# lambdaclass/ethrex

Measured on AMD Instinct MI355X. Metric: bn254_msm_point_adds_per_s, higher is better.
Workload: dtype u64x4_mod_bn254; 1 GPU; bn254_g1_msm_2^24; n_points=16777216, window_c=17, windows=15, signed_digits=True, parallelism=single GPU

## Files before the change

ethrex_amd/csrc/api_msm_bn254.hip:

```cpp
#include "msm_api_impl.h"

extern "C" int ethrex_mi355_msm_plan_create(size_t n, em_msm_plan **plan) {
    return msm_create_t(n, (msm_plan_t<Bn254G1> **)plan);
}
extern "C" int ethrex_mi355_msm_plan_destroy(em_msm_plan *p) {
    return msm_destroy_t((msm_plan_t<Bn254G1> *)p);
}
extern "C" int ethrex_mi355_msm_upload_points(em_msm_plan *p,
                                              const uint8_t *points64) {
    return msm_upload_points_t((msm_plan_t<Bn254G1> *)p, points64);
}
extern "C" int ethrex_mi355_msm_gen_points(em_msm_plan *p, uint64_t start) {
    return msm_gen_points_t((msm_plan_t<Bn254G1> *)p, start);
}
extern "C" int ethrex_mi355_msm_download_points(em_msm_plan *p, uint8_t *out64) {
    return msm_download_points_t((msm_plan_t<Bn254G1> *)p, out64);
}
extern "C" int ethrex_mi355_msm_upload_scalars(em_msm_plan *p,
                                               const uint8_t *scalars32) {
    return msm_upload_scalars_t((msm_plan_t<Bn254G1> *)p, scalars32);
}
extern "C" int ethrex_mi355_msm_run(em_msm_plan *p, uint8_t out[64]) {
    return msm_run_inner_t((msm_plan_t<Bn254G1> *)p, out, 0);
}
// ... 22 lines not shown
extern "C" int ethrex_mi355_msm_fb_info(em_msm_plan *p, int *c,
                                        double *precompute_ms,
                                        uint64_t *table_bytes) {
    if (!p) return EM_ERR_INPUT;
    if (c) *c = p->fb_c;
    if (precompute_ms) *precompute_ms = p->fb_precompute_ms;
    if (table_bytes) *table_bytes = p->fb_table_bytes;
    return EM_OK;
}

extern "C" int ethrex_mi355_msm_download_fb_rows(em_msm_plan *p, int w,
                                                 size_t start, size_t count,
                                                 uint8_t *out64) {
    if (!p || !out64 || !p->fb_c || !p->have_points || w < 0 ||
        w >= (254 + p->fb_c - 1) / p->fb_c || count == 0 || start >= p->n ||
        count > p->n - start)
        return EM_ERR_INPUT;
    int rc0 = msm_sync_t((msm_plan_t<Bn254G1> *)p);
    if (rc0) return rc0;
    hipLaunchKernelGGL(k_points_to_be, dim3(blocks_for(count, 256)), dim3(256),
                       0, 0, p->d_pts_ext + (size_t)w * p->n + start,
                       p->d_inf + start, p->d_scratch, count);
    HIP_TRY(hipMemcpy(out64, p->d_scratch, count * 64, hipMemcpyDeviceToHost));
    return EM_OK;
}

extern "C" int ethrex_mi355_msm_combine(em_msm_plan *p,
                                        const uint8_t *jacobians96,
                                        size_t count, uint8_t out[64]) {
    if (!p || !jacobians96 || !out || count == 0 || count * 96 > p->n * 64)
        return EM_ERR_INPUT;
    HIP_TRY(hipMemcpy(p->d_scratch, jacobians96, 96 * count,
                      hipMemcpyHostToDevice));
    hipLaunchKernelGGL((k_g1_combine<Bn254G1>), dim3(1), dim3(64), 0, 0,
                       p->d_scratch, count, p->sb[0].out);
    HIP_TRY(hipMemcpy(out, p->sb[0].out, 64, hipMemcpyDeviceToHost));
    return EM_OK;
}

extern "C" int ethrex_mi355_bn254_g1_msm(const uint8_t *points64,
                                         const uint8_t *scalars32, size_t n,
                                         uint8_t out[64]) {
    if (!points64 || !scalars32 || !out || n == 0) return EM_ERR_INPUT;
    em_msm_plan *p = nullptr;
    int rc = ethrex_mi355_msm_plan_create(n, &p);
    if (rc) return rc;
// ... 77 lines not shown
```

ethrex_amd/csrc/msm_api_impl.h:

```cpp
#pragma once
#include "em_api_common.h"

#include <rocprim/rocprim.hpp>

#include "../../include/ethrex_mi355.h"
#include "gpu_field.h"
#include "gpu_g1_9.h"
#include "msm_kernels.h"
#include "msm_fbm_partition_kernels.h"

using namespace em;


struct msm_step_bufs {
    uint32_t *keys_out = nullptr;
    uint32_t *vals_out = nullptr;
    uint32_t *offsets = nullptr;
    uint32_t *sched = nullptr;
    uint8_t *out = nullptr;
};

template <typename C>
struct msm_plan_t {
    using F = typename C::F;
    static constexpr int PB = pt_bytes<C>::AFF;
    static constexpr int JB = pt_bytes<C>::JAC;
    static constexpr int AB = PB;
    static constexpr int SB = msm_curve<C>::BN_SCALARS ? 254 : 256;
    size_t n;
    int cbits;
    g1aT<C> *d_pts = nullptr;
    g1aT<C> *d_pts_ext = nullptr;
    bool fixed_base = false;
    int fb_c = 0;
    uint32_t fb_chunk = 0;
    int fb_len_bits = 0;
    double fb_precompute_ms = 0;
    uint64_t fb_table_bytes = 0;
    uint32_t *d_fb_boff = nullptr;
    g1jT<C> *d_fb_slots = nullptr;
    uint32_t fbp_tile = 0;
    uint32_t *d_fbp = nullptr;
    uint8_t *d_inf = nullptr;
    fe4 *d_scalars = nullptr;
    uint8_t *d_scratch = nullptr;
    uint32_t *d_keys = nullptr;
    uint32_t *d_vals = nullptr;
    msm_step_bufs sb[2];
    void *d_sort_tmp = nullptr;
    size_t sort_tmp_bytes = 0;
    uint32_t *d_blen = nullptr;
    uint32_t *d_blen_out = nullptr;
    uint32_t *d_bids = nullptr;
    g1jT<C> *d_buckets = nullptr;
    g1jT<C> *d_seg_sum = nullptr;
    g1jT<C> *d_seg_wsum = nullptr;
    g1jT<C> *d_partials = nullptr;
    g1jT<C> *d_windows = nullptr;
    uint32_t *d_err = nullptr;
    bool use_tree = false;
    int tree_levels = 0;
    g1aT<C> *d_lvl[2] = {nullptr, nullptr};
    feL<F::L> *d_aux = nullptr;
    uint32_t *d_loff[2] = {nullptr, nullptr};
    uint32_t *d_cnt = nullptr;
// ... 21 lines not shown
    int apar = 0;
};

constexpr int NWIN_MAX = 32;

template <typename C>
static int msm_sync_t(msm_plan_t<C> *p);
template <typename C>
static void host_windows_horner(const uint8_t *wire, int nwin, int cbits,
                                uint8_t *out, int out_mode);

template <typename C>
static int msm_destroy_t(msm_plan_t<C> *p) {
    if (!p) return EM_ERR_INPUT;
    if (p->s_comp) {
        (void)hipStreamSynchronize(p->s_sort);
        (void)hipStreamSynchronize(p->s_comp);
    }
    (void)hipFree(p->d_pts);
    (void)hipFree(p->d_pts_ext);
    (void)hipFree(p->d_fb_boff);
    (void)hipFree(p->d_fb_slots);
    (void)hipFree(p->d_fbp);
    (void)hipFree(p->d_inf);
    (void)hipFree(p->d_scalars);
    (void)hipFree(p->d_scratch);
    (void)hipFree(p->d_keys);
    (void)hipFree(p->d_vals);
    (void)hipFree(p->d_sort_tmp);
    (void)hipFree(p->d_blen);
    (void)hipFree(p->d_blen_out);
    (void)hipFree(p->d_bids);
    (void)hipFree(p->d_buckets);
    (void)hipFree(p->d_seg_sum);
    (void)hipFree(p->d_seg_wsum);
    (void)hipFree(p->d_partials);
    (void)hipFree(p->d_windows);
    (void)hipFree(p->d_err);
    (void)hipFree(p->d_lvl[0]);
    (void)hipFree(p->d_lvl[1]);
    (void)hipFree(p->d_aux);
    (void)hipFree(p->d_loff[0]);
    (void)hipFree(p->d_loff[1]);
    (void)hipFree(p->d_cnt);
    (void)hipFree(p->d_scan_tmp);
    for (auto &b : p->sb) {
        (void)hipFree(b.keys_out);
        (void)hipFree(b.vals_out);
        (void)hipFree(b.offsets);
        (void)hipFree(b.sched);
        (void)hipFree(b.out);
    }
    if (p->h_out[0]) (void)hipHostFree(p->h_out[0]);
    if (p->h_out[1]) (void)hipHostFree(p->h_out[1]);
    for (int i = 0; i < 2; i++) {
        if (p->gx_sort[i]) (void)hipGraphExecDestroy(p->gx_sort[i]);
        if (p->gx_comp[i]) (void)hipGraphExecDestroy(p->gx_comp[i]);
    }
    if (p->s_sort) (void)hipStreamDestroy(p->s_sort);
    if (p->s_comp) (void)hipStreamDestroy(p->s_comp);
    delete p;
    return EM_OK;
}

constexpr int FBM_DEFAULT_C = 22;
constexpr size_t FBM_MIN_N = (size_t)1 << 23;

struct fbp_layout {
    size_t cnt_a, cnt_b, off_a, off_b, ucnt, uoff, words;
};
static inline fbp_layout fbp_lay(uint32_t nbuckets) {
    const size_t na = (size_t)(nbuckets >> 16) + 1;
    const size_t nc = (size_t)(nbuckets >> 8) + 1;
    fbp_layout l;
    l.cnt_a = 0;
    l.cnt_b = na;
    l.off_a = na + nc;
    l.off_b = 2 * na + nc;
    l.ucnt = 2 * na + 2 * nc;
    l.uoff = 2 * na + 3 * nc;
    l.words = 2 * na + 4 * nc;
    return l;
}
static inline size_t fbp_words(uint32_t nbuckets) { return fbp_lay(nbuckets).words; }

template <typename FN>
static int fbm_dispatch(int c, FN fn) {
    switch (c) {
    case 20: return fn(CfgFbm20{});
    case 22: return fn(CfgFbm22{});
    case 24: return fn(CfgFbm24{});
    }
    return EM_ERR_INPUT;
}

template <typename C>
static int fbm_select(size_t n) {
    if constexpr (!msm_curve<C>::FB_MERGED) {
        return 0;
    } else {
        int c = 0;
        if (const char *ev = std::getenv("EM_MSM_FB")) {
            c = atoi(ev);
            if (c != 20 && c != 22 && c != 24) return 0;
        } else if (n >= FBM_MIN_N && std::getenv("EM_MSM_TREE") == nullptr) {
            c = FBM_DEFAULT_C;
        } else {
// ... 116 lines not shown
    mal((void **)&p->d_keys, total * kb);
    mal((void **)&p->d_vals, total * 4);
    for (auto &b : p->sb) {
        mal((void **)&b.keys_out, total * kb);
        mal((void **)&b.vals_out, total * 4);
        mal((void **)&b.offsets, (nsched + 1) * 4);
        mal((void **)&b.sched, nsched * 4);
        mal((void **)&b.out, (size_t)NWIN_MAX * msm_plan_t<C>::JB);
    }
    mal((void **)&p->d_blen, nsched * 4);
    mal((void **)&p->d_blen_out, nsched * 4);
    mal((void **)&p->d_bids, nsched * 4);
    mal((void **)&p->d_buckets, (size_t)nbuckets * sizeof(g1jT<C>));
    if constexpr (msm_curve<C>::FB_MERGED) if (p->fb_c) {
        mal((void **)&p->d_fb_boff, ((size_t)nbuckets + 1) * 4);
        mal((void **)&p->d_fb_slots, nsched * sizeof(g1jT<C>));
        mal((void **)&p->d_cnt, ((size_t)nbuckets + 1) * 4);
        mal((void **)&p->d_loff[0], ((size_t)nbuckets + 1) * 4);
        mal((void **)&p->d_loff[1], ((size_t)nbuckets + 1) * 4);
        if (e == hipSuccess)
            e = rocprim::exclusive_scan(nullptr, p->scan_tmp_bytes, p->d_cnt,
                                        p->d_loff[0], 0u,
                                        (size_t)nbuckets + 1);
        if (e == hipSuccess) e = hipMalloc(&p->d_scan_tmp, p->scan_tmp_bytes);
        if (p->fbp_tile) mal((void **)&p->d_fbp, fbp_words(nbuckets) * 4);
    }
    mal((void **)&p->d_seg_sum, (size_t)nseg_tot * sizeof(g1jT<C>));
    mal((void **)&p->d_seg_wsum, (size_t)nseg_tot * sizeof(g1jT<C>));
    mal((void **)&p->d_partials, (size_t)npart * sizeof(g1jT<C>));
    mal((void **)&p->d_windows, (size_t)nwin * sizeof(g1jT<C>));
    mal((void **)&p->d_err, 4);
    if (e == hipSuccess) {
        if (p->keys16)
            e = rocprim::radix_sort_pairs(
                nullptr, p->sort_tmp_bytes, (const uint16_t *)p->d_keys,
                (uint16_t *)p->sb[0].keys_out, p->d_vals, p->sb[0].vals_out,
                n, 0, 16);
        else
            e = rocprim::radix_sort_pairs(
                nullptr, p->sort_tmp_bytes, p->d_keys, p->sb[0].keys_out,
                p->d_vals, p->sb[0].vals_out, total, 0, sort_bits);
        size_t tmp_len = 0;
        if (e == hipSuccess)
            e = rocprim::radix_sort_pairs(nullptr, tmp_len, p->d_blen,
                                          p->d_blen_out, p->d_bids,
                                          p->sb[0].sched, nsched, 0, 32);
        if (tmp_len > p->sort_tmp_bytes) p->sort_tmp_bytes = tmp_len;
        if (e == hipSuccess) e = hipMalloc(&p->d_sort_tmp, p->sort_tmp_bytes);
// ... 290 lines not shown
#define EM_HT(call)                         \
    do {                                    \
        hipError_t _e = (call);             \
        if (_e != hipSuccess) return _e;    \
    } while (0)

template <typename C, typename CFG>
static const g1aT<C> *msm_walk_pts(const msm_plan_t<C> *p) {
    constexpr bool TABLE = std::is_same_v<CFG, CfgFB> || is_fbm<CFG>::value;
    return TABLE ? p->d_pts_ext : p->d_pts;
}

static int msm_split_pct() {
    static int pct = std::getenv("EM_MSM_SPLIT")
                         ? atoi(std::getenv("EM_MSM_SPLIT"))
                         : 0;
    return pct;
}

template <typename C, typename CFG>
static hipError_t fbm_enqueue_partition(msm_plan_t<C> *p, int par,
                                        hipStream_t st) {
    using G = fbp_geom<CFG::IB>;
    const msm_step_bufs &b = p->sb[par];
    const size_t total = p->n * (size_t)CFG::NWIN_REAL;
    const uint32_t T = p->fbp_tile;
    const fbp_layout l = fbp_lay(G::NBUCKETS);
    uint32_t *cnt_a = p->d_fbp + l.cnt_a, *cnt_b = p->d_fbp + l.cnt_b;
    uint32_t *off_a = p->d_fbp + l.off_a, *off_b = p->d_fbp + l.off_b;
    uint32_t *ucnt = p->d_fbp + l.ucnt, *uoff = p->d_fbp + l.uoff;
    uint32_t *cnt_c = p->d_cnt;
    uint16_t *k16 = (uint16_t *)p->d_keys;
    uint8_t *k8 = (uint8_t *)p->d_keys + total * 2;
    uint32_t *v1 = p->d_vals, *v2 = b.keys_out;
    auto scan = [&](uint32_t *in, uint32_t *out, size_t len) {
        size_t stmp = p->scan_tmp_bytes;
        return rocprim::exclusive_scan(p->d_scan_tmp, stmp, in, out, 0u, len,
                                       rocprim::plus<uint32_t>(), st);
    };
    auto units = [&](const uint32_t *off, uint32_t regions) {
        hipLaunchKernelGGL((k_fbp_unit_counts<CFG>),
                           dim3(blocks_for((size_t)regions + 1, 256)),
                           dim3(256), 0, st, off, regions, T, ucnt);
        return scan(ucnt, uoff, (size_t)regions + 1);
    };
    const uint32_t nab = (uint32_t)(l.off_a - l.cnt_a);
    hipLaunchKernelGGL((k_fbp_zero<CFG>), dim3(blocks_for(nab, 256)),
                       dim3(256), 0, st, cnt_a, nab);
    hipLaunchKernelGGL((k_fbp_zero<CFG>),
                       dim3(blocks_for((size_t)G::NBUCKETS + 1, 256)),
                       dim3(256), 0, st, cnt_c, G::NBUCKETS + 1);
    hipLaunchKernelGGL((k_fbp_count_a<CFG>),
                       dim3(blocks_for(p->n, FBP_BLOCK * FBP_A_SPT)),
                       dim3(FBP_BLOCK), 0, st, p->d_scalars, p->d_inf, p->n,
                       cnt_a);
    EM_HT(scan(cnt_a, off_a, (size_t)G::NBIN_A + 1));
    hipLaunchKernelGGL((k_fbp_scatter_a<CFG>),
                       dim3(blocks_for(p->n, FBP_BLOCK)), dim3(FBP_BLOCK), 0,
                       st, p->d_scalars, p->d_inf, p->n, cnt_a, off_a, k16, v1);
    EM_HT(units(off_a, G::NREG_B));
    const dim3 grid_b(fbp_grid(total, T, G::NREG_B));
    hipLaunchKernelGGL((k_fbp_count<uint16_t, FBP_SHIFT_B>), grid_b,
                       dim3(FBP_BLOCK), 0, st, k16, off_a, uoff, G::NREG_B, T,
                       cnt_b);
    EM_HT(scan(cnt_b, off_b, (size_t)G::NREG_C + 1));
    hipLaunchKernelGGL((k_fbp_scatter<uint16_t, uint8_t, FBP_SHIFT_B, true>),
                       grid_b, dim3(FBP_BLOCK), (size_t)T * 6, st, k16, v1,
                       off_a, uoff, G::NREG_B, T, cnt_b, off_b, k8, v2);
    EM_HT(units(off_b, G::NREG_C));
    const dim3 grid_c(fbp_grid(total, T, G::NREG_C));
    hipLaunchKernelGGL((k_fbp_count<uint8_t, FBP_SHIFT_C>), grid_c,
                       dim3(FBP_BLOCK), 0, st, k8, off_b, uoff, G::NREG_C, T,
                       cnt_c);
    EM_HT(scan(cnt_c, p->d_fb_boff, (size_t)G::NBUCKETS + 1));
    hipLaunchKernelGGL((k_fbp_scatter<uint8_t, uint8_t, FBP_SHIFT_C, false>),
                       grid_c, dim3(FBP_BLOCK), (size_t)T * 5, st, k8, v2,
                       off_b, uoff, G::NREG_C, T, cnt_c, p->d_fb_boff,
                       (uint8_t *)nullptr, b.vals_out);
    return hipSuccess;
}

template <typename C, typename CFG>
static hipError_t msm_enqueue_sort_chain(msm_plan_t<C> *p, int par,
                                         hipStream_t st) {
    const msm_step_bufs &b = p->sb[par];
    size_t tmp = p->sort_tmp_bytes;
    if constexpr (is_fbm<CFG>::value) {
        const size_t total = p->n * (size_t)CFG::NWIN_REAL;
        constexpr uint32_t NB = CFG::NBUCKETS, NS = CFG::NSLOT;
        uint32_t *coff = p->d_loff[par];
        if (p->fbp_tile) {
            EM_HT((fbm_enqueue_partition<C, CFG>(p, par, st)));
        } else {
            hipLaunchKernelGGL((k_fbm_digits<CFG>),
                               dim3(blocks_for(p->n, 256)), dim3(256), 0, st,
                               p->d_scalars, p->d_inf, p->d_keys, p->d_vals,
                               p->n);
            EM_HT(rocprim::radix_sort_pairs(p->d_sort_tmp, tmp, p->d_keys,
                                            b.keys_out, p->d_vals, b.vals_out,
                                            total, 0, CFG::SORT_BITS, st));
            hipLaunchKernelGGL((k_offsets<CFG>),
// ... 343 lines not shown
```

ethrex_amd/csrc/msm_fbm_partition.h:

```cpp
#pragma once
#include <stddef.h>
#include <stdint.h>

#include "msm_fb_recode.h"

namespace em {

constexpr uint32_t FBP_TILE_MAX = 8192;
constexpr uint32_t FBP_TILE_DEFAULT = 4096;

template <int IB_>
struct fbp_geom {
    static_assert(IB_ > 16 && IB_ - 16 <= 8, "pass A takes 1..8 bits");
    static constexpr int IB = IB_;
    static constexpr int BITS_A = IB - 16;
    static constexpr uint32_t NBIN_A = 1u << BITS_A;
    static constexpr uint32_t NREG_B = NBIN_A;
    static constexpr uint32_t NREG_C = 1u << (IB - 8);
    static constexpr uint32_t NBUCKETS = 1u << IB;
};

constexpr int FBP_SHIFT_A = 16, FBP_SHIFT_B = 8, FBP_SHIFT_C = 0;
template <int SHIFT>
EM_FBM_HD uint32_t fbp_bin(uint32_t key) {
    return key >> SHIFT;
}
template <int SHIFT>
EM_FBM_HD uint32_t fbp_low(uint32_t key) {
    return key & ((1u << SHIFT) - 1u);
}

EM_FBM_HD uint32_t fbp_units(uint32_t len, uint32_t T) {
    return (len + T - 1) / T;
}

inline uint32_t fbp_grid(size_t total, uint32_t T, uint32_t regions) {
    return (uint32_t)(total / T) + regions + 1;
}

EM_FBM_HD uint32_t fbp_region_of(const uint32_t *uoff, uint32_t regions,
                                 uint32_t u) {
    uint32_t lo = 0, hi = regions;
    while (lo < hi) {
        uint32_t mid = (lo + hi + 1) >> 1;
        if (uoff[mid] <= u)
            lo = mid;
        else
            hi = mid - 1;
    }
    return lo;
}

EM_FBM_HD void fbp_unit_range(const uint32_t *off, const uint32_t *uoff,
                              uint32_t r, uint32_t u, uint32_t T, uint32_t &lo,
                              uint32_t &hi) {
    uint32_t end = off[r + 1];
    lo = off[r] + (u - uoff[r]) * T;
    hi = end - lo > T ? lo + T : end;
}

}
```

ethrex_amd/csrc/msm_fbm_partition_kernels.h:

```cpp
#pragma once
#include <hip/hip_runtime.h>

#include "msm_fbm_partition.h"
#include "msm_kernels.h"

namespace em {

constexpr int FBP_BLOCK = 256;
constexpr int FBP_A_SPT = 4;

template <typename CFG>
static __global__ void k_fbp_zero(uint32_t *__restrict__ p, uint32_t n) {
    uint32_t i = blockIdx.x * blockDim.x + threadIdx.x;
    if (i < n) p[i] = 0;
}

__device__ __forceinline__ uint32_t fbp_block_scan(uint32_t v, uint32_t *wsum) {
    const uint32_t lane = threadIdx.x & 63u, wave = threadIdx.x >> 6;
    uint32_t x = v;
#pragma unroll
    for (int d = 1; d < 64; d <<= 1) {
        uint32_t y = __shfl_up(x, d);
        if (lane >= (uint32_t)d) x += y;
    }
    if (lane == 63) wsum[wave] = x;
    __syncthreads();
    uint32_t add = 0;
    for (uint32_t k = 0; k < wave; k++) add += wsum[k];
    return add + x - v;
}

template <typename CFG>
__device__ __forceinline__ void fbp_entries(const fe4 &k, bool skip, size_t n,
                                            size_t i, uint32_t *key,
                                            uint32_t *val) {
    uint32_t carry = 0;
#pragma unroll
    for (int w = 0; w < CFG::NWIN_REAL; w++) {
        uint32_t neg;
        uint32_t mag =
            fbm_recode_step<CFG::C>(fbm_digit<CFG::C>(k.v, w), carry, neg);
        bool sk = skip || mag == 0;
        size_t e = (size_t)w * n + i;
        key[w] = sk ? 0u : mag - 1;
        val[w] = (uint32_t)e | (neg << 31) | (sk ? SGN_SKIP : 0u);
    }
}

template <typename CFG>
__global__ void __launch_bounds__(FBP_BLOCK)
k_fbp_count_a(const fe4 *__restrict__ scalars, const uint8_t *__restrict__ inf,
              size_t n, uint32_t *__restrict__ cnt) {
    using G = fbp_geom<CFG::IB>;
    constexpr int NW = CFG::NWIN_REAL;
    __shared__ uint32_t lh[G::NBIN_A];
    const uint32_t t = threadIdx.x;
    if (t < G::NBIN_A) lh[t] = 0;
    __syncthreads();
    size_t base = (size_t)blockIdx.x * (FBP_BLOCK * FBP_A_SPT);
    for (int s = 0; s < FBP_A_SPT; s++) {
        size_t i = base + (size_t)s * FBP_BLOCK + t;
        if (i >= n) break;
        uint32_t key[NW], val[NW];
        fbp_entries<CFG>(scalars[i], inf[i] != 0, n, i, key, val);
#pragma unroll
        for (int w = 0; w < NW; w++) atomicAdd(&lh[fbp_bin<FBP_SHIFT_A>(key[w])], 1u);
    }
    __syncthreads();
    if (t < G::NBIN_A && lh[t]) atomicAdd(&cnt[t], lh[t]);
}

template <typename CFG>
__global__ void __launch_bounds__(FBP_BLOCK)
k_fbp_scatter_a(const fe4 *__restrict__ scalars,
                const uint8_t *__restrict__ inf, size_t n,
                uint32_t *__restrict__ cnt, const uint32_t *__restrict__ off,
                uint16_t *__restrict__ kout, uint32_t *__restrict__ vout) {
    using G = fbp_geom<CFG::IB>;
    constexpr int NW = CFG::NWIN_REAL;
    constexpr int E = FBP_BLOCK * NW;
    __shared__ uint32_t lv[E];
    __shared__ uint16_t lk[E];
    __shared__ uint8_t lb[E];
    __shared__ uint32_t lh[G::NBIN_A], lcur[G::NBIN_A], ldelta[G::NBIN_A];
    __shared__ uint32_t wsum[FBP_BLOCK / 64];
    const uint32_t t = threadIdx.x;
    if (t < G::NBIN_A) lh[t] = 0;
    __syncthreads();
    const size_t first = (size_t)blockIdx.x * FBP_BLOCK;
    const size_t i = first + t;
    const bool valid = i < n;
    uint32_t key[NW], val[NW];
    if (valid) {
        fbp_entries<CFG>(scalars[i], inf[i] != 0, n, i, key, val);
#pragma unroll
        for (int w = 0; w < NW; w++) atomicAdd(&lh[fbp_bin<FBP_SHIFT_A>(key[w])], 1u);
    }
    __syncthreads();
    const uint32_t mine = t < G::NBIN_A ? lh[t] : 0u;
    const uint32_t ex = fbp_block_scan(mine, wsum);
    if (t < G::NBIN_A) {
        lcur[t] = ex;
        if (mine) ldelta[t] = off[t] + (atomicSub(&cnt[t], mine) - mine) - ex;
    }
    __syncthreads();
    if (valid) {
#pragma unroll
        for (int w = 0; w < NW; w++) {
            uint32_t b = fbp_bin<FBP_SHIFT_A>(key[w]);
            uint32_t pos = atomicAdd(&lcur[b], 1u);
            lv[pos] = val[w];
            lk[pos] = (uint16_t)fbp_low<FBP_SHIFT_A>(key[w]);
            lb[pos] = (uint8_t)b;
        }
    }
    __syncthreads();
    const size_t left = n - first;
    const uint32_t cntv =
        (uint32_t)(left < (size_t)FBP_BLOCK ? left : (size_t)FBP_BLOCK) * NW;
    for (uint32_t j = t; j < cntv; j += FBP_BLOCK) {
        uint32_t dst = ldelta[lb[j]] + j;
        vout[dst] = lv[j];
        kout[dst] = lk[j];
    }
}

template <typename CFG>
static __global__ void k_fbp_unit_counts(const uint32_t *__restrict__ off,
                                         uint32_t regions, uint32_t T,
                                         uint32_t *__restrict__ ucnt) {
    uint32_t r = blockIdx.x * blockDim.x + threadIdx.x;
    if (r > regions) return;
    ucnt[r] = r == regions ? 0u : fbp_units(off[r + 1] - off[r], T);
}

template <typename KIN, int SHIFT>
__global__ void __launch_bounds__(FBP_BLOCK)
k_fbp_count(const KIN *__restrict__ kin, const uint32_t *__restrict__ off,
            const uint32_t *__restrict__ uoff, uint32_t regions, uint32_t T,
            uint32_t *__restrict__ cnt) {
    __shared__ uint32_t lh[256];
    const uint32_t t = threadIdx.x, u = blockIdx.x;
    if (u >= uoff[regions]) return;
    const uint32_t r = fbp_region_of(uoff, regions, u);
    uint32_t lo, hi;
    fbp_unit_range(off, uoff, r, u, T, lo, hi);
    lh[t] = 0;
    __syncthreads();
    for (uint32_t j = lo + t; j < hi; j += FBP_BLOCK)
        atomicAdd(&lh[fbp_bin<SHIFT>((uint32_t)kin[j])], 1u);
    __syncthreads();
    if (lh[t]) atomicAdd(&cnt[r * 256u + t], lh[t]);
}

template <typename KIN, typename KOUT, int SHIFT, bool WRITE_KEYS>
__global__ void __launch_bounds__(FBP_BLOCK)
k_fbp_scatter(const KIN *__restrict__ kin, const uint32_t *__restrict__ vin,
              const uint32_t *__restrict__ off,
              const uint32_t *__restrict__ uoff, uint32_t regions, uint32_t T,
              uint32_t *__restrict__ cnt, const uint32_t *__restrict__ boff,
              KOUT *__restrict__ kout, uint32_t *__restrict__ vout) {
    extern __shared__ __align__(16) unsigned char fbp_dyn[];
    uint32_t *lv = reinterpret_cast<uint32_t *>(fbp_dyn);
    KIN *lk = reinterpret_cast<KIN *>(lv + T);
    __shared__ uint32_t lh[256], lcur[256], ldelta[256];
    __shared__ uint32_t wsum[FBP_BLOCK / 64];
    const uint32_t t = threadIdx.x, u = blockIdx.x;
    if (u >= uoff[regions]) return;
    const uint32_t r = fbp_region_of(uoff, regions, u);
    uint32_t lo, hi;
    fbp_unit_range(off, uoff, r, u, T, lo, hi);
    lh[t] = 0;
    __syncthreads();
    for (uint32_t j = lo + t; j < hi; j += FBP_BLOCK)
        atomicAdd(&lh[fbp_bin<SHIFT>((uint32_t)kin[j])], 1u);
    __syncthreads();
    const uint32_t mine = lh[t];
    const uint32_t ex = fbp_block_scan(mine, wsum);
    lcur[t] = ex;
    if (mine) {
        const uint32_t g = r * 256u + t;
        ldelta[t] = boff[g] + (atomicSub(&cnt[g], mine) - mine) - ex;
    }
    __syncthreads();
    for (uint32_t j = lo + t; j < hi; j += FBP_BLOCK) {
        KIN k = kin[j];
        uint32_t pos = atomicAdd(&lcur[fbp_bin<SHIFT>((uint32_t)k)], 1u);
        lv[pos] = vin[j];
        lk[pos] = k;
    }
    __syncthreads();
    const uint32_t len = hi - lo;
    for (uint32_t j = t; j < len; j += FBP_BLOCK) {
        KIN k = lk[j];
        uint32_t dst = ldelta[fbp_bin<SHIFT>((uint32_t)k)] + j;
        vout[dst] = lv[j];
        if constexpr (WRITE_KEYS)
            kout[dst] = (KOUT)fbp_low<SHIFT>((uint32_t)k);
    }
}

}
```

ethrex_amd/lib.py:

```python
import array
import ctypes
import os

_DIR = os.path.dirname(os.path.abspath(__file__))
_SO = os.path.join(_DIR, "libethrex_mi355.so")

if not os.path.exists(_SO):
    raise ImportError(
        f"HIP core library missing: {_SO}. Run __graft_entry__.build() "
        "(hipcc --offload-arch=gfx950). The product path has no CPU fallback.")

_lib = ctypes.CDLL(_SO)

EM_OK = 0
EM_ERR_POINT = 1
EM_ERR_INPUT = 2
EM_ERR_HIP = 3

_lib.ethrex_mi355_version.restype = ctypes.c_char_p
_lib.ethrex_mi355_last_error.restype = ctypes.c_char_p
for _f in ("device_count", "set_device", "bn254_g1_add", "bn254_g1_mul",
           "bn254_g1_msm", "bn254_fr_ntt", "bn254_g1_combine",
           "msm_plan_create", "msm_plan_destroy", "msm_upload_points",
           "msm_gen_points", "msm_download_points", "msm_upload_scalars",
           "msm_run", "msm_run_partial", "msm_run_async", "msm_sync",
           "msm_run_partial_async", "msm_wait_one", "bn254_g1_combine_cpu",
           "msm_last_times", "msm_combine", "msm_scalars_from_ntt",
           "msm_fb_info", "msm_download_fb_rows", "ntt_device_data",
           "ntt_plan_create", "ntt_plan_destroy", "ntt_upload", "ntt_run",
           "ntt_download", "ntt_last_times", "ntt_fill_from_digests",
           "ntt_last_fill_ms", "keccak_device_digests",
           "ntt_run_coset", "bn254_fr_coset_ntt", "quot_plan_create",
           "quot_plan_destroy", "quot_upload", "quot_load_device",
           "quot_mul_ab_into_c", "quot_run", "quot_download",
           "quot_device_data", "quot_last_times", "r1cs_plan_create",
           "r1cs_plan_destroy", "r1cs_upload_matrix", "r1cs_upload_witness",
           "r1cs_witness_from_device", "r1cs_eval", "r1cs_download",
           "r1cs_device_data", "r1cs_last_times"):
    getattr(_lib, f"ethrex_mi355_{_f}").restype = ctypes.c_int


class HipCoreError(RuntimeError):
    def __init__(self, rc, what):
        self.rc = rc
        super().__init__(f"{what}: rc={rc} ({last_error()})")


def _check(rc, what):
    if rc != EM_OK:
        raise HipCoreError(rc, what)


def _buf(b):
    return (ctypes.c_uint8 * len(b)).from_buffer_copy(b)


def version() -> str:
    return _lib.ethrex_mi355_version().decode()


def last_error() -> str:
    return (_lib.ethrex_mi355_last_error() or b"").decode()


# ... 131 lines not shown
    def last_times(self):
        t = (ctypes.c_double * 5)()
        self._call("last_times", t)
        return {"digits_sort_ms": t[0], "bucket_acc_ms": t[1],
                "reduce_ms": t[2], "combine_ms": t[3], "total_ms": t[4]}

    def destroy(self):
        if self._p:
            self._fn("plan_destroy")(self._p)
            self._p = ctypes.c_void_p()

    def __del__(self):
        try:
            self.destroy()
        except Exception:
            pass


class MsmPlan(_MsmPlanBase):

    _PREFIX, _AFF, _JAC = "msm", 64, 96
    _OPS = _MsmPlanBase._OPS + (
        "fb_info", "download_fb_rows", "run_partial_async", "wait_one",
        "scalars_from_ntt", "combine")

    def last_times(self):
        t = super().last_times()
        t["fb_precompute_ms"] = self._fb_info()[1]
        return t

    def _fb_info(self):
        c = ctypes.c_int(0)
        ms = ctypes.c_double(0.0)
        nbytes = ctypes.c_uint64(0)
        self._call("fb_info", ctypes.byref(c), ctypes.byref(ms),
                   ctypes.byref(nbytes))
        return c.value, ms.value, nbytes.value

    @property
    def fixed_base(self) -> int:
        return self._fb_info()[0]

    @property
    def fb_table_bytes(self) -> int:
        return self._fb_info()[2]

    def download_fb_rows(self, w: int, start: int, count: int) -> bytes:
        out = (ctypes.c_uint8 * (64 * count))()
        self._call("download_fb_rows", ctypes.c_int(w),
                   ctypes.c_size_t(start), ctypes.c_size_t(count), out)
        return bytes(out)

    def run_partial_async(self):
        self._pending.append(self._call_out("run_partial_async", self._JAC))

    def wait_one(self) -> bytes:
        if not self._pending:
            return b""
        self._call("wait_one")
        return bytes(self._pending.pop(0))

    def scalars_from_ntt(self, ntt_plan, offset: int = 0):
        self._scalars_from_ntt(ntt_plan, offset)

    def combine(self, jacobians: bytes, count: int) -> bytes:
        out = (ctypes.c_uint8 * 64)()
        self._call("combine", _buf(jacobians), ctypes.c_size_t(count), out)
        return bytes(out)


class NttPlan:
    def __init__(self, n: int):
        self.n = n
        self._p = ctypes.c_void_p()
# ... 463 lines not shown
```

include/ethrex_mi355.h:

```cpp
#ifndef ETHREX_MI355_H
#define ETHREX_MI355_H

#include <stddef.h>
#include <stdint.h>

#ifdef __cplusplus
extern "C" {
#endif

enum {
    EM_OK = 0,
    EM_ERR_POINT = 1,
    EM_ERR_INPUT = 2,
    EM_ERR_HIP = 3,
};

const char *ethrex_mi355_version(void);
int ethrex_mi355_device_count(int *count);
int ethrex_mi355_set_device(int device);
const char *ethrex_mi355_last_error(void);

int ethrex_mi355_bn254_g1_add(const uint8_t p1[64], const uint8_t p2[64],
                              uint8_t out[64]);
int ethrex_mi355_bn254_g1_mul(const uint8_t point[64], const uint8_t scalar[32],
// ... 9 lines not shown
int ethrex_mi355_msm_plan_create(size_t n, em_msm_plan **plan);
int ethrex_mi355_msm_plan_destroy(em_msm_plan *plan);
int ethrex_mi355_msm_upload_points(em_msm_plan *plan, const uint8_t *points64);
int ethrex_mi355_msm_gen_points(em_msm_plan *plan, uint64_t start);
int ethrex_mi355_msm_download_points(em_msm_plan *plan, uint8_t *out64);
int ethrex_mi355_msm_upload_scalars(em_msm_plan *plan, const uint8_t *scalars32);
int ethrex_mi355_msm_run(em_msm_plan *plan, uint8_t out[64]);
int ethrex_mi355_msm_run_partial(em_msm_plan *plan, uint8_t out[96]);
int ethrex_mi355_msm_run_async(em_msm_plan *plan, uint8_t out[64]);
int ethrex_mi355_msm_sync(em_msm_plan *plan);
int ethrex_mi355_msm_run_partial_async(em_msm_plan *plan, uint8_t out[96]);
int ethrex_mi355_msm_wait_one(em_msm_plan *plan);
int ethrex_mi355_bn254_g1_combine(const uint8_t *jacobians96, size_t count,
                                  uint8_t out[64]);
int ethrex_mi355_bn254_g1_combine_cpu(const uint8_t *jacobians96,
                                      size_t count, uint8_t out[64]);
int ethrex_mi355_msm_scalars_from_ntt(em_msm_plan *plan, const void *ntt_data,
                                      uint64_t offset);
int ethrex_mi355_msm_last_times(em_msm_plan *plan, double times_ms[5]);
int ethrex_mi355_msm_fb_info(em_msm_plan *plan, int *c, double *precompute_ms,
                             uint64_t *table_bytes);
int ethrex_mi355_msm_download_fb_rows(em_msm_plan *plan, int w, size_t start,
                                      size_t count, uint8_t *out64);
int ethrex_mi355_msm_combine(em_msm_plan *plan, const uint8_t *jacobians96,
                             size_t count, uint8_t out[64]);

typedef struct em_mpt em_mpt;
int ethrex_mi355_mpt_create(const uint8_t *keys32, const uint8_t *vals,
                            const uint64_t *val_offs, size_t n, em_mpt **out);
int ethrex_mi355_mpt_destroy(em_mpt *t);
int ethrex_mi355_mpt_max_depth(em_mpt *t, int *depth);
int ethrex_mi355_mpt_level_encode(em_mpt *t, int depth, uint8_t *buf,
                                  uint64_t *offs, size_t buf_cap,
                                  size_t max_n, size_t *n_hash);
int ethrex_mi355_mpt_level_set_hashes(em_mpt *t, int depth,
                                      const uint8_t *h32, size_t n_hash);
int ethrex_mi355_mpt_root(em_mpt *t, uint8_t out[32]);

typedef struct em_keccak_plan em_keccak_plan;
int ethrex_mi355_keccak256_batch(const uint8_t *msgs, const uint64_t *offsets,
                                 size_t n, uint8_t *out32);
int ethrex_mi355_keccak_plan_create(size_t max_bytes, size_t max_n,
                                    em_keccak_plan **plan);
int ethrex_mi355_keccak_plan_destroy(em_keccak_plan *plan);
int ethrex_mi355_keccak_upload(em_keccak_plan *plan, const uint8_t *msgs,
                               const uint64_t *offsets, size_t n);
// ... 147 lines not shown
```

Measured before the change: 12.87 billion point_adds/s.

## Use per-tile count matrix and scan for deterministic radix partition passes

The three-pass bucket partition used to count per bucket with global atomics and pick scatter offsets by atomicSub on those counts. It now writes each tile's histogram into a count matrix laid out bin-major by unit, runs an exclusive scan over the matrix, and derives region offsets with small offset kernels. Pass A also keys its bins by window, so every window's entries are placed in a fixed order. The aim is a stable, deterministic partition without contended global atomics or zeroing kernels, at the cost of extra memory and much larger scans over the matrices. A debug API that downloads the grouping result is added as well.

```diff
diff --git a/ethrex_amd/csrc/api_msm_bn254.hip b/ethrex_amd/csrc/api_msm_bn254.hip
--- a/ethrex_amd/csrc/api_msm_bn254.hip
+++ b/ethrex_amd/csrc/api_msm_bn254.hip
@@ -68,6 +68,26 @@
                        0, 0, p->d_pts_ext + (size_t)w * p->n + start,
                        p->d_inf + start, p->d_scratch, count);
     HIP_TRY(hipMemcpy(out64, p->d_scratch, count * 64, hipMemcpyDeviceToHost));
+    return EM_OK;
+}
+
+extern "C" int ethrex_mi355_msm_debug_grouping(em_msm_plan *p, uint32_t *vals,
+                                               size_t vals_cap, uint32_t *boff,
+                                               size_t boff_cap, size_t *n_vals,
+                                               size_t *n_boff) {
+    if (!p || !n_vals || !n_boff) return EM_ERR_INPUT;
+    *n_vals = *n_boff = 0;
+    if (!p->fb_c) return EM_OK;
+    int rc0 = msm_sync_t((msm_plan_t<Bn254G1> *)p);
+    if (rc0) return rc0;
+    *n_vals = p->n * (size_t)((254 + p->fb_c - 1) / p->fb_c);
+    *n_boff = ((size_t)1 << (p->fb_c - 1)) + 1;
+    if (vals && vals_cap >= *n_vals)
+        HIP_TRY(hipMemcpy(vals, p->sb[0].vals_out, *n_vals * 4,
+                          hipMemcpyDeviceToHost));
+    if (boff && boff_cap >= *n_boff)
+        HIP_TRY(hipMemcpy(boff, p->d_fb_boff, *n_boff * 4,
+                          hipMemcpyDeviceToHost));
     return EM_OK;
 }
 
diff --git a/ethrex_amd/csrc/msm_api_impl.h b/ethrex_amd/csrc/msm_api_impl.h
--- a/ethrex_amd/csrc/msm_api_impl.h
+++ b/ethrex_amd/csrc/msm_api_impl.h
@@ -41,6 +41,8 @@
     g1jT<C> *d_fb_slots = nullptr;
     uint32_t fbp_tile = 0;
     uint32_t *d_fbp = nullptr;
+    uint32_t *d_fbp_mat = nullptr;
+    uint32_t *d_fbp_scan = nullptr;
     uint8_t *d_inf = nullptr;
     fe4 *d_scalars = nullptr;
     uint8_t *d_scratch = nullptr;
@@ -108,6 +110,8 @@
     (void)hipFree(p->d_fb_boff);
     (void)hipFree(p->d_fb_slots);
     (void)hipFree(p->d_fbp);
+    (void)hipFree(p->d_fbp_mat);
+    (void)hipFree(p->d_fbp_scan);
     (void)hipFree(p->d_inf);
     (void)hipFree(p->d_scalars);
     (void)hipFree(p->d_scratch);
@@ -153,22 +157,28 @@
 constexpr size_t FBM_MIN_N = (size_t)1 << 23;
 
 struct fbp_layout {
-    size_t cnt_a, cnt_b, off_a, off_b, ucnt, uoff, words;
+    size_t off_a, off_b, ucnt, uoff, words;
 };
 static inline fbp_layout fbp_lay(uint32_t nbuckets) {
     const size_t na = (size_t)(nbuckets >> 16) + 1;
     const size_t nc = (size_t)(nbuckets >> 8) + 1;
     fbp_layout l;
-    l.cnt_a = 0;
-    l.cnt_b = na;
-    l.off_a = na + nc;
-    l.off_b = 2 * na + nc;
-    l.ucnt = 2 * na + 2 * nc;
-    l.uoff = 2 * na + 3 * nc;
-    l.words = 2 * na + 4 * nc;
+    l.off_a = 0;
+    l.off_b = na;
+    l.ucnt = na + nc;
+    l.uoff = na + 2 * nc;
+    l.words = na + 3 * nc;
     return l;
 }
 static inline size_t fbp_words(uint32_t nbuckets) { return fbp_lay(nbuckets).words; }
+
+static inline size_t fbp_mat_words(size_t n, size_t total, uint32_t T,
+                                   uint32_t nbuckets, uint32_t nwin) {
+    size_t a = fbp_mat_len_a(n, nbuckets >> 16, nwin);
+    size_t b = fbp_mat_len(total, T, nbuckets >> 16);
+    size_t c = fbp_mat_len(total, T, nbuckets >> 8);
+    return std::max(a, std::max(b, c));
+}
 
 template <typename FN>
 static int fbm_dispatch(int c, FN fn) {
@@ -331,8 +341,20 @@
             e = rocprim::exclusive_scan(nullptr, p->scan_tmp_bytes, p->d_cnt,
                                         p->d_loff[0], 0u,
                                         (size_t)nbuckets + 1);
+        if (p->fbp_tile) {
+            const size_t mw = fbp_mat_words(n, total, p->fbp_tile, nbuckets,
+                                            (uint32_t)(total / n));
+            mal((void **)&p->d_fbp, fbp_words(nbuckets) * 4);
+            mal((void **)&p->d_fbp_mat, mw * 4);
+            mal((void **)&p->d_fbp_scan, mw * 4);
+            size_t mtmp = 0;
+            if (e == hipSuccess)
+                e = rocprim::exclusive_scan(nullptr, mtmp, p->d_fbp_mat,
+                                            p->d_fbp_scan, 0u, mw);
+            if (mtmp > p->scan_tmp_bytes) p->scan_tmp_bytes = mtmp;
+            if (e == hipSuccess) e = hipMemset(p->d_fbp_mat, 0, mw * 4);
+        }
         if (e == hipSuccess) e = hipMalloc(&p->d_scan_tmp, p->scan_tmp_bytes);
-        if (p->fbp_tile) mal((void **)&p->d_fbp, fbp_words(nbuckets) * 4);
     }
     mal((void **)&p->d_seg_sum, (size_t)nseg_tot * sizeof(g1jT<C>));
     mal((void **)&p->d_seg_wsum, (size_t)nseg_tot * sizeof(g1jT<C>));
@@ -669,14 +691,14 @@
 static hipError_t fbm_enqueue_partition(msm_plan_t<C> *p, int par,
                                         hipStream_t st) {
     using G = fbp_geom<CFG::IB>;
+    constexpr uint32_t NW = CFG::NWIN_REAL;
     const msm_step_bufs &b = p->sb[par];
-    const size_t total = p->n * (size_t)CFG::NWIN_REAL;
+    const size_t total = p->n * (size_t)NW;
     const uint32_t T = p->fbp_tile;
     const fbp_layout l = fbp_lay(G::NBUCKETS);
-    uint32_t *cnt_a = p->d_fbp + l.cnt_a, *cnt_b = p->d_fbp + l.cnt_b;
     uint32_t *off_a = p->d_fbp + l.off_a, *off_b = p->d_fbp + l.off_b;
     uint32_t *ucnt = p->d_fbp + l.ucnt, *uoff = p->d_fbp + l.uoff;
-    uint32_t *cnt_c = p->d_cnt;
+    uint32_t *mat = p->d_fbp_mat, *msc = p->d_fbp_scan;
     uint16_t *k16 = (uint16_t *)p->d_keys;
     uint8_t *k8 = (uint8_t *)p->d_keys + total * 2;
     uint32_t *v1 = p->d_vals, *v2 = b.keys_out;
@@ -691,39 +713,42 @@
                            dim3(256), 0, st, off, regions, T, ucnt);
         return scan(ucnt, uoff, (size_t)regions + 1);
     };
-    const uint32_t nab = (uint32_t)(l.off_a - l.cnt_a);
-    hipLaunchKernelGGL((k_fbp_zero<CFG>), dim3(blocks_for(nab, 256)),
-                       dim3(256), 0, st, cnt_a, nab);
-    hipLaunchKernelGGL((k_fbp_zero<CFG>),
-                       dim3(blocks_for((size_t)G::NBUCKETS + 1, 256)),
-                       dim3(256), 0, st, cnt_c, G::NBUCKETS + 1);
+    auto offsets = [&](uint32_t regions, uint32_t *off_next) {
+        hipLaunchKernelGGL((k_fbp_offsets<CFG>),
+                           dim3(blocks_for((size_t)regions * 256 + 1, 256)),
+                           dim3(256), 0, st, msc, uoff, regions, off_next);
+    };
+    const uint32_t ua = (uint32_t)fbp_units_a(p->n);
     hipLaunchKernelGGL((k_fbp_count_a<CFG>),
                        dim3(blocks_for(p->n, FBP_BLOCK * FBP_A_SPT)),
                        dim3(FBP_BLOCK), 0, st, p->d_scalars, p->d_inf, p->n,
-                       cnt_a);
-    EM_HT(scan(cnt_a, off_a, (size_t)G::NBIN_A + 1));
-    hipLaunchKernelGGL((k_fbp_scatter_a<CFG>),
-                       dim3(blocks_for(p->n, FBP_BLOCK)), dim3(FBP_BLOCK), 0,
-                       st, p->d_scalars, p->d_inf, p->n, cnt_a, off_a, k16, v1);
+                       ua, mat);
+    EM_HT(scan(mat, msc, fbp_mat_len_a(p->n, G::NBIN_A, NW)));
+    hipLaunchKernelGGL((k_fbp_offsets_a<CFG>), dim3(1), dim3(256), 0, st, msc,
+                       ua, G::NBIN_A, off_a);
+    hipLaunchKernelGGL((k_fbp_scatter_a<CFG>), dim3(ua), dim3(FBP_BLOCK), 0,
+                       st, p->d_scalars, p->d_inf, p->n, ua, msc, k16, v1);
     EM_HT(units(off_a, G::NREG_B));
     const dim3 grid_b(fbp_grid(total, T, G::NREG_B));
     hipLaunchKernelGGL((k_fbp_count<uint16_t, FBP_SHIFT_B>), grid_b,
                        dim3(FBP_BLOCK), 0, st, k16, off_a, uoff, G::NREG_B, T,
-                       cnt_b);
-    EM_HT(scan(cnt_b, off_b, (size_t)G::NREG_C + 1));
+                       mat);
+    EM_HT(scan(mat, msc, fbp_mat_len(total, T, G::NREG_B)));
+    offsets(G::NREG_B, off_b);
     hipLaunchKernelGGL((k_fbp_scatter<uint16_t, uint8_t, FBP_SHIFT_B, true>),
                        grid_b, dim3(FBP_BLOCK), (size_t)T * 6, st, k16, v1,
-                       off_a, uoff, G::NREG_B, T, cnt_b, off_b, k8, v2);
+                       off_a, uoff, G::NREG_B, T, msc, k8, v2);
     EM_HT(units(off_b, G::NREG_C));
     const dim3 grid_c(fbp_grid(total, T, G::NREG_C));
     hipLaunchKernelGGL((k_fbp_count<uint8_t, FBP_SHIFT_C>), grid_c,
                        dim3(FBP_BLOCK), 0, st, k8, off_b, uoff, G::NREG_C, T,
-                       cnt_c);
-    EM_HT(scan(cnt_c, p->d_fb_boff, (size_t)G::NBUCKETS + 1));
+                       mat);
+    EM_HT(scan(mat, msc, fbp_mat_len(total, T, G::NREG_C)));
+    offsets(G::NREG_C, p->d_fb_boff);
     hipLaunchKernelGGL((k_fbp_scatter<uint8_t, uint8_t, FBP_SHIFT_C, false>),
                        grid_c, dim3(FBP_BLOCK), (size_t)T * 5, st, k8, v2,
-                       off_b, uoff, G::NREG_C, T, cnt_c, p->d_fb_boff,
-                       (uint8_t *)nullptr, b.vals_out);
+                       off_b, uoff, G::NREG_C, T, msc, (uint8_t *)nullptr,
+                       b.vals_out);
     return hipSuccess;
 }
 
diff --git a/ethrex_amd/csrc/msm_fbm_partition.h b/ethrex_amd/csrc/msm_fbm_partition.h
--- a/ethrex_amd/csrc/msm_fbm_partition.h
+++ b/ethrex_amd/csrc/msm_fbm_partition.h
@@ -8,6 +8,8 @@
 
 constexpr uint32_t FBP_TILE_MAX = 8192;
 constexpr uint32_t FBP_TILE_DEFAULT = 4096;
+constexpr uint32_t FBP_SA = 256;
+static_assert(FBP_SA == 256 || FBP_SA == 512 || FBP_SA == 1024, "pass-A unit");
 
 template <int IB_>
 struct fbp_geom {
@@ -28,6 +30,14 @@
 template <int SHIFT>
 EM_FBM_HD uint32_t fbp_low(uint32_t key) {
     return key & ((1u << SHIFT) - 1u);
+}
+
+EM_FBM_HD uint32_t fbp_bin_a(uint32_t key, uint32_t w, uint32_t nwin) {
+    return fbp_bin<FBP_SHIFT_A>(key) * nwin + w;
+}
+
+EM_FBM_HD size_t fbp_units_a(size_t n) {
+    return (n + FBP_SA - 1) / FBP_SA;
 }
 
 EM_FBM_HD uint32_t fbp_units(uint32_t len, uint32_t T) {
@@ -59,4 +69,28 @@
     hi = end - lo > T ? lo + T : end;
 }
 
+EM_FBM_HD size_t fbp_mat_a(uint32_t bin, size_t units, size_t unit) {
+    return (size_t)bin * units + unit;
 }
+
+EM_FBM_HD size_t fbp_mat(const uint32_t *uoff, uint32_t r, uint32_t bin,
+                         uint32_t u) {
+    return 256 * (size_t)uoff[r] + (size_t)bin * (uoff[r + 1] - uoff[r]) +
+           (u - uoff[r]);
+}
+
+EM_FBM_HD size_t fbp_mat_region(const uint32_t *uoff, uint32_t regions,
+                                uint32_t g) {
+    const uint32_t r = g >> 8;
+    if (r >= regions) return 256 * (size_t)uoff[regions];
+    return 256 * (size_t)uoff[r] + (size_t)(g & 255u) * (uoff[r + 1] - uoff[r]);
+}
+
+inline size_t fbp_mat_len_a(size_t n, uint32_t nbin_a, uint32_t nwin) {
+    return (size_t)nbin_a * nwin * fbp_units_a(n) + 1;
+}
+inline size_t fbp_mat_len(size_t total, uint32_t T, uint32_t regions) {
+    return 256 * (size_t)fbp_grid(total, T, regions) + 1;
+}
+
+}
diff --git a/ethrex_amd/csrc/msm_fbm_partition_kernels.h b/ethrex_amd/csrc/msm_fbm_partition_kernels.h
--- a/ethrex_amd/csrc/msm_fbm_partition_kernels.h
+++ b/ethrex_amd/csrc/msm_fbm_partition_kernels.h
@@ -8,12 +8,9 @@
 
 constexpr int FBP_BLOCK = 256;
 constexpr int FBP_A_SPT = 4;
-
-template <typename CFG>
-static __global__ void k_fbp_zero(uint32_t *__restrict__ p, uint32_t n) {
-    uint32_t i = blockIdx.x * blockDim.x + threadIdx.x;
-    if (i < n) p[i] = 0;
-}
+constexpr int FBP_A_UPB = FBP_BLOCK * FBP_A_SPT / (int)FBP_SA;
+constexpr int FBP_A_SPT_SC = (int)FBP_SA / FBP_BLOCK;
+static_assert(FBP_A_UPB >= 1 && FBP_A_SPT_SC >= 1, "pass-A unit vs block");
 
 __device__ __forceinline__ uint32_t fbp_block_scan(uint32_t v, uint32_t *wsum) {
     const uint32_t lane = threadIdx.x & 63u, wave = threadIdx.x >> 6;
@@ -50,79 +47,123 @@
 template <typename CFG>
 __global__ void __launch_bounds__(FBP_BLOCK)
 k_fbp_count_a(const fe4 *__restrict__ scalars, const uint8_t *__restrict__ inf,
-              size_t n, uint32_t *__restrict__ cnt) {
+              size_t n, uint32_t units, uint32_t *__restrict__ mat) {
     using G = fbp_geom<CFG::IB>;
     constexpr int NW = CFG::NWIN_REAL;
-    __shared__ uint32_t lh[G::NBIN_A];
+    constexpr uint32_t NB = G::NBIN_A * NW;
+    constexpr uint32_t UPB = FBP_A_UPB;
+    __shared__ uint32_t lh[UPB * NB];
     const uint32_t t = threadIdx.x;
-    if (t < G::NBIN_A) lh[t] = 0;
+    for (uint32_t j = t; j < UPB * NB; j += FBP_BLOCK) lh[j] = 0;
     __syncthreads();
     size_t base = (size_t)blockIdx.x * (FBP_BLOCK * FBP_A_SPT);
     for (int s = 0; s < FBP_A_SPT; s++) {
         size_t i = base + (size_t)s * FBP_BLOCK + t;
         if (i >= n) break;
+        uint32_t *h = lh + (uint32_t)(s * FBP_BLOCK) / FBP_SA * NB;
         uint32_t key[NW], val[NW];
         fbp_entries<CFG>(scalars[i], inf[i] != 0, n, i, key, val);
 #pragma unroll
-        for (int w = 0; w < NW; w++) atomicAdd(&lh[fbp_bin<FBP_SHIFT_A>(key[w])], 1u);
-    }
-    __syncthreads();
-    if (t < G::NBIN_A && lh[t]) atomicAdd(&cnt[t], lh[t]);
+        for (int w = 0; w < NW; w++) atomicAdd(&h[fbp_bin_a(key[w], w, NW)], 1u);
+    }
+    __syncthreads();
+    const uint32_t unit0 = blockIdx.x * UPB;
+    for (uint32_t j = t; j < UPB * NB; j += FBP_BLOCK) {
+        const uint32_t b = j / UPB, sub = j % UPB;
+        if (unit0 + sub < units)
+            mat[fbp_mat_a(b, units, unit0 + sub)] = lh[sub * NB + b];
+    }
 }
 
 template <typename CFG>
 __global__ void __launch_bounds__(FBP_BLOCK)
 k_fbp_scatter_a(const fe4 *__restrict__ scalars,
-                const uint8_t *__restrict__ inf, size_t n,
-                uint32_t *__restrict__ cnt, const uint32_t *__restrict__ off,
-                uint16_t *__restrict__ kout, uint32_t *__restrict__ vout) {
+                const uint8_t *__restrict__ inf, size_t n, uint32_t units,
+                const uint32_t *__restrict__ scan, uint16_t *__restrict__ kout,
+                uint32_t *__restrict__ vout) {
     using G = fbp_geom<CFG::IB>;
     constexpr int NW = CFG::NWIN_REAL;
-    constexpr int E = FBP_BLOCK * NW;
+    constexpr uint32_t NB = G::NBIN_A * NW;
+    constexpr uint32_t BPT = (NB + FBP_BLOCK - 1) / FBP_BLOCK;
+    constexpr int SPT = FBP_A_SPT_SC;
+    constexpr uint32_t E = FBP_SA * NW;
     __shared__ uint32_t lv[E];
     __shared__ uint16_t lk[E];
-    __shared__ uint8_t lb[E];
-    __shared__ uint32_t lh[G::NBIN_A], lcur[G::NBIN_A], ldelta[G::NBIN_A];
+    __shared__ uint16_t lb[E];
+    __shared__ uint32_t lcur[NB], ldelta[NB];
     __shared__ uint32_t wsum[FBP_BLOCK / 64];
-    const uint32_t t = threadIdx.x;
-    if (t < G::NBIN_A) lh[t] = 0;
-    __syncthreads();
-    const size_t first = (size_t)blockIdx.x * FBP_BLOCK;
-    const size_t i = first + t;
-    const bool valid = i < n;
-    uint32_t key[NW], val[NW];
-    if (valid) {
-        fbp_entries<CFG>(scalars[i], inf[i] != 0, n, i, key, val);
-#pragma unroll
-        for (int w = 0; w < NW; w++) atomicAdd(&lh[fbp_bin<FBP_SHIFT_A>(key[w])], 1u);
-    }
-    __syncthreads();
-    const uint32_t mine = t < G::NBIN_A ? lh[t] : 0u;
-    const uint32_t ex = fbp_block_scan(mine, wsum);
-    if (t < G::NBIN_A) {
-        lcur[t] = ex;
-        if (mine) ldelta[t] = off[t] + (atomicSub(&cnt[t], mine) - mine) - ex;
-    }
-    __syncthreads();
-    if (valid) {
-#pragma unroll
-        for (int w = 0; w < NW; w++) {
-            uint32_t b = fbp_bin<FBP_SHIFT_A>(key[w]);
-            uint32_t pos = atomicAdd(&lcur[b], 1u);
-            lv[pos] = val[w];
-            lk[pos] = (uint16_t)fbp_low<FBP_SHIFT_A>(key[w]);
-            lb[pos] = (uint8_t)b;
+    const uint32_t t = threadIdx.x, unit = blockIdx.x;
+    for (uint32_t j = t; j < NB; j += FBP_BLOCK) lcur[j] = 0;
+    __syncthreads();
+    const size_t first = (size_t)unit * FBP_SA;
+    fe4 k[SPT];
+    bool skip[SPT];
+#pragma unroll
+    for (int s = 0; s < SPT; s++) {
+        const size_t i = first + (size_t)s * FBP_BLOCK + t;
+        if (i < n) {
+            k[s] = scalars[i];
+            skip[s] = inf[i] != 0;
+            uint32_t key[NW], val[NW];
+            fbp_entries<CFG>(k[s], skip[s], n, i, key, val);
+#pragma unroll
+            for (int w = 0; w < NW; w++)
+                atomicAdd(&lcur[fbp_bin_a(key[w], w, NW)], 1u);
+        }
+    }
+    __syncthreads();
+    uint32_t c[BPT], mine = 0;
+#pragma unroll
+    for (uint32_t q = 0; q < BPT; q++) {
+        const uint32_t b = t * BPT + q;
+        c[q] = b < NB ? lcur[b] : 0u;
+        mine += c[q];
+    }
+    uint32_t ex = fbp_block_scan(mine, wsum);
+#pragma unroll
+    for (uint32_t q = 0; q < BPT; q++) {
+        const uint32_t b = t * BPT + q;
+        if (b < NB) {
+            lcur[b] = ex;
+            ldelta[b] = scan[fbp_mat_a(b, units, unit)] - ex;
+            ex += c[q];
+        }
+    }
+    __syncthreads();
+#pragma unroll
+    for (int s = 0; s < SPT; s++) {
+        const size_t i = first + (size_t)s * FBP_BLOCK + t;
+        if (i < n) {
+            uint32_t key[NW], val[NW];
+            fbp_entries<CFG>(k[s], skip[s], n, i, key, val);
+#pragma unroll
+            for (int w = 0; w < NW; w++) {
+                uint32_t b = fbp_bin_a(key[w], w, NW);
+                uint32_t pos = atomicAdd(&lcur[b], 1u);
+                lv[pos] = val[w];
+                lk[pos] = (uint16_t)fbp_low<FBP_SHIFT_A>(key[w]);
+                lb[pos] = (uint16_t)b;
+            }
         }
     }
     __syncthreads();
     const size_t left = n - first;
     const uint32_t cntv =
-        (uint32_t)(left < (size_t)FBP_BLOCK ? left : (size_t)FBP_BLOCK) * NW;
+        (uint32_t)(left < (size_t)FBP_SA ? left : (size_t)FBP_SA) * NW;
     for (uint32_t j = t; j < cntv; j += FBP_BLOCK) {
         uint32_t dst = ldelta[lb[j]] + j;
         vout[dst] = lv[j];
         kout[dst] = lk[j];
     }
+}
+
+template <typename CFG>
+static __global__ void k_fbp_offsets_a(const uint32_t *__restrict__ scan,
+                                       uint32_t units, uint32_t nreg,
+                                       uint32_t *__restrict__ off) {
+    uint32_t h = blockIdx.x * blockDim.x + threadIdx.x;
+    if (h > nreg) return;
+    off[h] = scan[fbp_mat_a(h * CFG::NWIN_REAL, units, 0)];
 }
 
 template <typename CFG>
@@ -138,7 +179,7 @@
 __global__ void __launch_bounds__(FBP_BLOCK)
 k_fbp_count(const KIN *__restrict__ kin, const uint32_t *__restrict__ off,
             const uint32_t *__restrict__ uoff, uint32_t regions, uint32_t T,
-            uint32_t *__restrict__ cnt) {
+            uint32_t *__restrict__ mat) {
     __shared__ uint32_t lh[256];
     const uint32_t t = threadIdx.x, u = blockIdx.x;
     if (u >= uoff[regions]) return;
@@ -150,7 +191,17 @@
     for (uint32_t j = lo + t; j < hi; j += FBP_BLOCK)
         atomicAdd(&lh[fbp_bin<SHIFT>((uint32_t)kin[j])], 1u);
     __syncthreads();
-    if (lh[t]) atomicAdd(&cnt[r * 256u + t], lh[t]);
+    mat[fbp_mat(uoff, r, t, u)] = lh[t];
+}
+
+template <typename CFG>
+static __global__ void k_fbp_offsets(const uint32_t *__restrict__ scan,
+                                     const uint32_t *__restrict__ uoff,
+                                     uint32_t regions,
+                                     uint32_t *__restrict__ off_next) {
+    uint32_t g = blockIdx.x * blockDim.x + threadIdx.x;
+    if (g > regions * 256u) return;
+    off_next[g] = scan[fbp_mat_region(uoff, regions, g)];
 }
 
 template <typename KIN, typename KOUT, int SHIFT, bool WRITE_KEYS>
@@ -158,8 +209,8 @@
 k_fbp_scatter(const KIN *__restrict__ kin, const uint32_t *__restrict__ vin,
               const uint32_t *__restrict__ off,
               const uint32_t *__restrict__ uoff, uint32_t regions, uint32_t T,
-              uint32_t *__restrict__ cnt, const uint32_t *__restrict__ boff,
-              KOUT *__restrict__ kout, uint32_t *__restrict__ vout) {
+              const uint32_t *__restrict__ scan, KOUT *__restrict__ kout,
+              uint32_t *__restrict__ vout) {
     extern __shared__ __align__(16) unsigned char fbp_dyn[];
     uint32_t *lv = reinterpret_cast<uint32_t *>(fbp_dyn);
     KIN *lk = reinterpret_cast<KIN *>(lv + T);
@@ -178,10 +229,7 @@
     const uint32_t mine = lh[t];
     const uint32_t ex = fbp_block_scan(mine, wsum);
     lcur[t] = ex;
-    if (mine) {
-        const uint32_t g = r * 256u + t;
-        ldelta[t] = boff[g] + (atomicSub(&cnt[g], mine) - mine) - ex;
-    }
+    ldelta[t] = scan[fbp_mat(uoff, r, t, u)] - ex;
     __syncthreads();
     for (uint32_t j = lo + t; j < hi; j += FBP_BLOCK) {
         KIN k = kin[j];
diff --git a/ethrex_amd/lib.py b/ethrex_amd/lib.py
--- a/ethrex_amd/lib.py
+++ b/ethrex_amd/lib.py
@@ -26,7 +26,8 @@
            "msm_run", "msm_run_partial", "msm_run_async", "msm_sync",
            "msm_run_partial_async", "msm_wait_one", "bn254_g1_combine_cpu",
            "msm_last_times", "msm_combine", "msm_scalars_from_ntt",
-           "msm_fb_info", "msm_download_fb_rows", "ntt_device_data",
+           "msm_fb_info", "msm_download_fb_rows", "msm_debug_grouping",
+           "ntt_device_data",
            "ntt_plan_create", "ntt_plan_destroy", "ntt_upload", "ntt_run",
            "ntt_download", "ntt_last_times", "ntt_fill_from_digests",
            "ntt_last_fill_ms", "keccak_device_digests",
@@ -40,6 +41,9 @@
     getattr(_lib, f"ethrex_mi355_{_f}").restype = ctypes.c_int
 
 
+FBM_PARTITION_SA = 256
+
+
 class HipCoreError(RuntimeError):
     def __init__(self, rc, what):
         self.rc = rc
@@ -217,7 +221,7 @@
     _PREFIX, _AFF, _JAC = "msm", 64, 96
     _OPS = _MsmPlanBase._OPS + (
         "fb_info", "download_fb_rows", "run_partial_async", "wait_one",
-        "scalars_from_ntt", "combine")
+        "scalars_from_ntt", "combine", "debug_grouping")
 
     def last_times(self):
         t = super().last_times()
@@ -245,6 +249,19 @@
         self._call("download_fb_rows", ctypes.c_int(w),
                    ctypes.c_size_t(start), ctypes.c_size_t(count), out)
         return bytes(out)
+
+    def debug_grouping(self):
+        nv, nb = ctypes.c_size_t(0), ctypes.c_size_t(0)
+        self._call("debug_grouping", None, ctypes.c_size_t(0), None,
+                   ctypes.c_size_t(0), ctypes.byref(nv), ctypes.byref(nb))
+        if nv.value == 0:
+            return b"", b""
+        vals = (ctypes.c_uint32 * nv.value)()
+        boff = (ctypes.c_uint32 * nb.value)()
+        self._call("debug_grouping", vals, ctypes.c_size_t(nv.value), boff,
+                   ctypes.c_size_t(nb.value), ctypes.byref(nv),
+                   ctypes.byref(nb))
+        return bytes(vals), bytes(boff)
 
     def run_partial_async(self):
         self._pending.append(self._call_out("run_partial_async", self._JAC))
diff --git a/include/ethrex_mi355.h b/include/ethrex_mi355.h
--- a/include/ethrex_mi355.h
+++ b/include/ethrex_mi355.h
@@ -55,6 +55,10 @@
                              uint64_t *table_bytes);
 int ethrex_mi355_msm_download_fb_rows(em_msm_plan *plan, int w, size_t start,
                                       size_t count, uint8_t *out64);
+int ethrex_mi355_msm_debug_grouping(em_msm_plan *plan, uint32_t *vals,
+                                    size_t vals_cap, uint32_t *boff,
+                                    size_t boff_cap, size_t *n_vals,
+                                    size_t *n_boff);
 int ethrex_mi355_msm_combine(em_msm_plan *plan, const uint8_t *jacobians96,
                              size_t count, uint8_t out[64]);
 
```

Result: slower. 12.13 billion point_adds/s (-5.7%).
